# Quyans/SG-NeRF

Measured on AMD Instinct MI355X. Metric: rays/sec + ms/frame, 800×800×64 samples, ScanNet scene, 1/2/4/8 GPU, higher is better.
Workload: dtype f32 (3xf16 split MFMA, fp32 accumulate); 1 GPU; synth-room 800x800 rays x SR=64 samples, D=400, K=8, P=26, 1200000 neural points (BASELINE config 2, 1 frame per rank per step); rays_per_frame=640000, SR=64, K=8, D=400, points=1200000, parallelism=frame-sharded x1, outputs=rgb, ray mask, background transmission, coarse_point_opacity [R, SR]

## Files before the change

sg-nerf_amd/csrc/mlp_x3.hip:

```cpp
#include <cstdio>
#include <cstdlib>
#include <algorithm>
#include <cmath>
#include <utility>
#include <vector>

#include "agg_device.h"
#include "x3_split.h"

namespace sgn {
namespace {
namespace x3 {

constexpr int NW16 = 8, TPB16 = NW16 * 64;
constexpr int PAIR = 2048;
constexpr int SLOT_PAIRS = 32;
constexpr int SLOT = SLOT_PAIRS * PAIR;
constexpr int NSLOT = 2;
constexpr int PD = 2;
constexpr size_t PROJ_BYTES_PER_POINT = HID * 4;
struct XL {
    int ks, tp, np, kc;
    uint32_t off;
};
__host__ __device__ constexpr int nch(XL l) { return (l.ks + l.kc - 1) / l.kc; }
__host__ __device__ constexpr int nk(XL l, int c) { return l.ks - c * l.kc < l.kc ? l.ks - c * l.kc : l.kc; }

template <class Net>
struct Sched {
    static constexpr int layer_chunks(int l) { return Net::L[l].np * nch(Net::L[l]); }
    static constexpr int base(int l) { return l == 0 ? 0 : base(l - 1) + layer_chunks(l - 1); }
    static constexpr int total() { return base(Net::NL); }
    static constexpr int idx(int l, int p, int c) { return base(l) + p * nch(Net::L[l]) + c; }
    static constexpr int cl(int n, int l = 0) { return (l + 1 >= Net::NL || n < base(l + 1)) ? l : cl(n, l + 1); }
    static constexpr int cp(int n) { return (n - base(cl(n))) / nch(Net::L[cl(n)]); }
    static constexpr int cc(int n) { return (n - base(cl(n))) % nch(Net::L[cl(n)]); }
    static constexpr uint32_t off(int n) {
        return Net::L[cl(n)].off +
               (uint32_t)((cp(n) * Net::L[cl(n)].ks + cc(n) * Net::L[cl(n)].kc) * Net::L[cl(n)].tp) * PAIR;
    }
    static constexpr int pairs(int n) { return nk(Net::L[cl(n)], cc(n)) * Net::L[cl(n)].tp; }
};
struct X3B {
    h8 hi, lo;
};

__device__ __forceinline__ X3B split8(const float (&v)[8]) {
    const X3Pair p = split8_unit(v);
    return X3B{p.hi, p.lo};
}

__device__ __forceinline__ float lrelu_x3(float a) {
    float r = 0.01f * a;
    asm("v_max_f32 %0, %1, %0" : "+v"(r) : "v"(a));
    return r;
}
__device__ __forceinline__ X3B lrelu_split8(const float (&a)[8], float inv) {
    float v[8];
#pragma unroll
    for (int j = 0; j < 8; ++j) v[j] = lrelu_x3(a[j] * inv);
    return split8(v);
}

__device__ __forceinline__ void lds_dma_1k(const WBlob &wb, char *dst, int w, int lane, uint32_t soff) {
    asm volatile("" : "+s"(soff));
    __builtin_amdgcn_raw_ptr_buffer_load_lds(wb.rsrc, (__attribute__((address_space(3))) void *)(dst + w * 1024), 16,
                                             lane * 16 + w * 1024, soff, 0, 0);
}

template <class Net, int N, int NWv = NW16>
__device__ __forceinline__ void dma_chunk(const WBlob &wb, char *dst, int w, int lane, int) {
    using S = Sched<Net>;
    constexpr int nf = 2 * S::pairs(N);
    static_for<(nf + NWv - 1) / NWv>([&](auto jj) {
        constexpr int J = decltype(jj)::value;
        const int i = w + NWv * J;
        if (NWv * (J + 1) <= nf || i < nf)
            lds_dma_1k(wb, dst + NWv * J * 1024, w, lane, S::off(N) + (uint32_t)(NWv * J * 1024));
    });
}

template <class Net, int N, int J, int NWv = NW16>
__device__ __forceinline__ void dma_piece(const WBlob &wb, char *dst, int w, int lane, int) {
    using S = Sched<Net>;
    constexpr int nf = 2 * S::pairs(N);
    constexpr int PW = (nf + NWv - 1) / NWv;
    const int i = w * PW + J;
    if (nf % NWv == 0 || i < nf) {
        uint32_t soff = S::off(N) + (uint32_t)((J & ~3) * 1024);
        asm volatile("" : "+s"(soff));
        __builtin_amdgcn_raw_ptr_buffer_load_lds(wb.rsrc,
                                                 (__attribute__((address_space(3))) void *)(dst + (w * PW + (J & ~3)) * 1024),
                                                 16, lane * 16 + w * PW * 1024, soff, (J & 3) * 1024, 0);
    }
}
template <class Net, int N, int NWv = NW16>
constexpr int dma_pieces() { return (2 * Sched<Net>::pairs(N) + NWv - 1) / NWv; }

__device__ __forceinline__ int cur_slot(int s) { return s; }
__device__ __forceinline__ int dma_slot(int s) { return s ^ 1; }
__device__ __forceinline__ void chunk_exit(int &s, int) { s ^= 1; }

template <class Net, int N, int NWv = NW16, int VM = 0>
__device__ __forceinline__ void chunk_enter(const WBlob &, char *, int, int, int, int) {
    static_assert(VM >= 0 && VM < 64, "vmcnt range");
    if constexpr (VM == 0)
        asm volatile("s_waitcnt vmcnt(0)" ::: "memory");
    else
        __builtin_amdgcn_s_waitcnt((VM & 15) | (7 << 4) | (15 << 8) | ((VM >> 4) << 14));
    asm volatile("s_waitcnt lgkmcnt(0)" ::: "memory");
    __builtin_amdgcn_s_barrier();
}

struct NoHook {
    template <class C>
    __device__ void operator()(C) const {}
};
struct VmZero {
    static constexpr int vm(int) { return 0; }
};


template <int F>
__device__ __forceinline__ void sincos_f(float x, float &s, float &c) {
    sincos_acc(x * (float)(1 << F), s, c);
}
constexpr uint32_t OFF16_BASE = 0;
constexpr uint32_t OFF16_W0B = OFF16_BASE;
constexpr uint32_t OFF16_W1 = OFF16_W0B + 32 * PAIR;
constexpr uint32_t OFF16_W2 = OFF16_W1 + 128 * PAIR;
constexpr uint32_t OFF16_W3 = OFF16_W2 + 144 * PAIR;
constexpr uint32_t OFF16_W0A = OFF16_W3 + 128 * PAIR;
constexpr uint32_t OFF16_WB = OFF16_W0A + 112 * PAIR;
constexpr uint32_t OFF16_C0 = OFF16_WB + 176 * PAIR;
constexpr uint32_t OFF16_C1 = OFF16_C0 + 72 * PAIR;
constexpr uint32_t OFF16_C2 = OFF16_C1 + 32 * PAIR;
constexpr uint32_t OFF16_F32 = OFF16_C2 + 32 * PAIR;
constexpr int Y_B0 = 0, Y_B1 = 256, Y_B2 = 512, Y_B3 = 768, Y_WA = 1024, Y_BB = 1280, Y_BA = 1536, Y_INV = 1537;
constexpr int Y_CB0 = Y_INV + 8 + 3, Y_CB1 = Y_CB0 + 128, Y_CB2 = Y_CB1 + 128, Y_CW3 = Y_CB2 + 128, Y_CB3 = Y_CW3 + 384;
constexpr int N_Y32 = Y_CB3 + 4;
constexpr size_t BLOB_BYTES_ALL = OFF16_F32 + (size_t)N_Y32 * 4;
__host__ __device__ constexpr size_t blob_bytes_sg(int) { return BLOB_BYTES_ALL; }
static_assert(N_Y32 % 4 == 0, "fp32 section in 16-B units");

constexpr int NWR = 4;
constexpr int NSLR = NSLOT;
static_assert(NWR == 4, "row workgroup: 4 waves");
template <int SP_>
struct NetR16T {
    static constexpr int NW = NWR, SP = SP_;
    static constexpr int KC = SP_ / 16;
    static constexpr int NL = 4;
    static constexpr XL L[NL] = {{2, 16, 1, KC, OFF16_W0B}, {8, 16, 1, KC, OFF16_W1}, {9, 16, 1, KC, OFF16_W2},
                                 {8, 8, 2, 2 * KC, OFF16_W3}};
};
template <int KB, int SP_>
struct NetR16SGT {
    static constexpr int NW = NWR, SP = SP_;
    static constexpr int KC = SP_ / 16;
    static constexpr int NL = 5;
    static constexpr XL L[NL] = {{2, 16, 1, KC, OFF16_W0B}, {8, 16, 1, KC, OFF16_W1}, {KB, 16, 1, KC, OFF16_WB},
                                 {9, 16, 1, KC, OFF16_W2}, {8, 8, 2, 2 * KC, OFF16_W3}};
};
struct NetProj16 {
    static constexpr int NW = NW16, SP = SLOT_PAIRS;
    static constexpr int NL = 1;
    static constexpr XL L[NL] = {{7, 16, 1, 2, OFF16_W0A}};
};
constexpr int NWC = 8, SPC = NWC == 4 ? 16 : 32, KCC = SPC / 8;
static_assert(NWC == 4 || NWC == 8, "colour workgroup: 4 or 8 waves");
struct NetColor16 {
    static constexpr int NW = NWC, SP = SPC;
    static constexpr int NL = 3;
    static constexpr XL L[NL] = {{9, 8, 1, KCC, OFF16_C0}, {4, 8, 1, KCC, OFF16_C1}, {4, 8, 1, KCC, OFF16_C2}};
};
static_assert(Sched<NetR16T<16>>::total() == 27 && Sched<NetR16T<32>>::total() == 14 &&
                  Sched<NetR16T<32>>::pairs(9) == 16, "16x16 row stream");
static_assert(NWC == 4 ? Sched<NetColor16>::total() == 9 && Sched<NetColor16>::pairs(4) == 8
                       : Sched<NetColor16>::total() == 5 && Sched<NetColor16>::pairs(2) == 8, "16x16 colour stream");

__device__ __forceinline__ f32x4 mfma16(h8 a, h8 b, f32x4 c) {
    return __builtin_amdgcn_mfma_f32_16x16x32_f16(a, b, c, 0, 0, 0);
}

template <int NS>
struct X3S {
    X3B b[NS];
};

template <class Net, int L, bool TRANS = false, class Vm = VmZero, int P = 0, int AOFF = 0, bool PIPE = false,
          int NS, int NA, class SlotT, class InFn, class PostFn = NoHook, class EndFn = NoHook, class MidFn = NoHook>
__device__ __forceinline__ void run_layer_ns(const WBlob &wb, char *lds, SlotT &slot, int w, int lane, int lz,
                                             f32x4 (&acc)[NS][NA], InFn &&in, PostFn &&post = PostFn{},
                                             EndFn &&end = EndFn{}, MidFn &&mid = MidFn{}) {
    constexpr XL ly = Net::L[L];
    constexpr int TP = ly.tp;
    static_assert((TP == 16 || TP == 8) && P < ly.np, "passes of 16 or 8 output tiles");
    static_assert(AOFF + TP <= NA, "accumulator view");
    X3S<NS> Bn;
    if constexpr (PIPE) Bn = in(std::integral_constant<int, 0>{});
    static_for<nch(ly)>([&](auto cc) {
        constexpr int C = decltype(cc)::value;
        constexpr int N = Sched<Net>::idx(L, P, C), NN = (N + 1) % Sched<Net>::total();
        constexpr int NWv = Net::NW, SLOTv = Net::SP * PAIR;
        static_assert(nk(ly, C) * TP <= Net::SP, "chunk larger than a ring slot");
        chunk_enter<Net, N, NWv, Vm::vm(C)>(wb, lds, slot, w, lane, lz);
        post(cc);
        const char *sl = lds + cur_slot(slot) * SLOTv;
        char *dnext = lds + dma_slot(slot) * SLOTv;
        constexpr int NF = nk(ly, C) * TP;
        constexpr int PW = dma_pieces<Net, NN, NWv>();
        auto frag = [&](int f, int part) { return *(const h8 *)(sl + (2 * f + part) * 1024 + lane * 16); };
        h8 fh[PD], fl[PD];
#pragma unroll
        for (int f = 0; f < PD; ++f) {
            fh[f] = frag(f, 0);
            fl[f] = frag(f, 1);
        }
        __builtin_amdgcn_sched_group_barrier(0x100, 2 * PD, 0);
        static_for<nk(ly, C)>([&](auto kk) {
            constexpr int KK = decltype(kk)::value;
            constexpr int KS = C * ly.kc + KK;
            if constexpr (NS > 1 && KK > 0 && !PIPE) __builtin_amdgcn_sched_barrier(0);
            X3S<NS> B;
            if constexpr (PIPE) B = Bn;
            else B = in(std::integral_constant<int, KS>{});
            static_for<TP>([&](auto tt) {
                constexpr int t = decltype(tt)::value, F = KK * TP + t;
                const h8 Ah = fh[F % PD], Al = fl[F % PD];
                if constexpr (F + PD < NF) {
                    fh[F % PD] = frag(F + PD, 0);
                    fl[F % PD] = frag(F + PD, 1);
                }
#pragma unroll
                for (int s = 0; s < NS; ++s) {
                    f32x4 &c = acc[s][AOFF + t];
                    if constexpr (TRANS) {
                        c = mfma16(B.b[s].hi, Al, c);
                        c = mfma16(B.b[s].lo, Ah, c);
                        c = mfma16(B.b[s].hi, Ah, c);
                    } else {
                        c = mfma16(Al, B.b[s].hi, c);
                        c = mfma16(Ah, B.b[s].lo, c);
                        c = mfma16(Ah, B.b[s].hi, c);
                    }
                }
                constexpr int NSP = NF / 2 > 0 ? NF / 2 : 1;
                if constexpr (F < NSP) {
                    static_for<(F + 1) * PW / NSP - F * PW / NSP>([&](auto jj) {
                        dma_piece<Net, NN, F * PW / NSP + decltype(jj)::value, NWv>(wb, dnext, w, lane, lz);
                    });
                }
                mid(std::integral_constant<int, (C * ly.kc + KK) * TP + t>{});
                if constexpr (PIPE && t == TP / 2 - 1 && KS + 1 < ly.ks)
                    Bn = in(std::integral_constant<int, (KS + 1 < ly.ks ? KS + 1 : KS)>{});
                if constexpr (NS == 1) {
                    __builtin_amdgcn_sched_group_barrier(0x008, 1, 0);
                    __builtin_amdgcn_sched_group_barrier(0x100, 1, 0);
                    __builtin_amdgcn_sched_group_barrier(0x008, 1, 0);
                    __builtin_amdgcn_sched_group_barrier(0x100, 1, 0);
                    __builtin_amdgcn_sched_group_barrier(0x008, 1, 0);
                } else {
                    __builtin_amdgcn_sched_group_barrier(0x008, 3 * NS / 2, 0);
                    __builtin_amdgcn_sched_group_barrier(0x100, 1, 0);
                    __builtin_amdgcn_sched_group_barrier(0x008, 3 * NS - 3 * NS / 2, 0);
                    __builtin_amdgcn_sched_group_barrier(0x100, 1, 0);
                }
            });
        });
        __builtin_amdgcn_sched_barrier(0);
        end(cc);
        chunk_exit(slot, lane);
        __builtin_amdgcn_sched_barrier(0);
    });
}

template <class Net, int L, bool TRANS = false, class Vm = VmZero, int P = 0, class SlotT, class InFn,
          class PostFn = NoHook, class EndFn = NoHook, class MidFn = NoHook>
__device__ __forceinline__ void run_layer16(const WBlob &wb, char *lds, SlotT &slot, int w, int lane, int lz,
                                            f32x4 (&acc)[Net::L[L].tp], InFn &&in, PostFn &&post = PostFn{},
                                            EndFn &&end = EndFn{}, MidFn &&mid = MidFn{}) {
    constexpr int TP = Net::L[L].tp;
    run_layer_ns<Net, L, TRANS, Vm, P, 0>(wb, lds, slot, w, lane, lz, reinterpret_cast<f32x4(&)[1][TP]>(acc),
                                          [&](auto k) { return X3S<1>{{in(k)}}; }, post, end, mid);
}

template <bool ADD>
__device__ __forceinline__ void chain_out16(const f32x4 (&acc)[16], const f32x4 (&add)[16], float inv, X3B (&out)[8]) {
#pragma unroll
    for (int s = 0; s < 8; ++s) {
        float v[8];
#pragma unroll
        for (int j = 0; j < 8; ++j) {
            const float a = acc[2 * s + (j >> 2)][j & 3];
            const float y = ADD ? (a + add[2 * s + (j >> 2)][j & 3]) * inv : a * inv;
            v[j] = fmaxf(y, 0.01f * y);
        }
        out[s] = split8(v);
    }
}

struct Proj16Args {
    const float *emb;
    int64_t n;
    const void *blob;
    float *proj;
    const float *xyz, *color, *dir, *conf;
    float *rec;
    const int32_t *idx;
    const int64_t *n_dev;
};
constexpr int REC16_FLOATS = 16;
constexpr int Y_LDS_OFF = NSLOT * SLOT;
constexpr int PROJ16_LDS = Y_LDS_OFF + N_Y32 * 4;

__global__ __launch_bounds__(TPB16, 1) void k_point_proj16(Proj16Args a) {
    __shared__ __attribute__((aligned(16))) char lds[PROJ16_LDS];
    const int lane = threadIdx.x & 63, g = lane >> 4;
    const int w = __builtin_amdgcn_readfirstlane(threadIdx.x >> 6);
    const WBlob wb = make_blob(a.blob, BLOB_BYTES_ALL);
    {
        const float *src = (const float *)((const char *)a.blob + OFF16_F32);
        float *dst = (float *)(lds + Y_LDS_OFF);
        for (int i = threadIdx.x; i < N_Y32; i += TPB16) dst[i] = src[i];
    }
    __syncthreads();
    int slot = 0;
    dma_chunk<NetProj16, 0, NW16>(wb, lds, w, lane, 0);
    const int64_t n = a.idx ? min(*a.n_dev, a.n) : a.n;
    const int64_t ntile = (n + 16 * NW16 - 1) / (16 * NW16);
    for (int64_t tile = blockIdx.x; tile < ntile; tile += gridDim.x) {
        int lz = 0;
        asm volatile("" : "+s"(lz));
        const float *Yl = (const float *)(lds + lz + Y_LDS_OFF);
        const int64_t j = tile * (16 * NW16) + w * 16 + (lane & 15);
        const bool ok = j < n;
        const int64_t p = a.idx ? (ok ? (int64_t)a.idx[j] : 0) : j;
        float f8[8];
        {
            const f32x4 *e4 = (const f32x4 *)(a.emb + (ok ? p : 0) * 32 + 8 * g);
            const f32x4 u0 = e4[0], u1 = e4[1];
            f8[0] = u0[0]; f8[1] = u0[1]; f8[2] = u0[2]; f8[3] = u0[3];
            f8[4] = u1[0]; f8[5] = u1[1]; f8[6] = u1[2]; f8[7] = u1[3];
        }
        f32x4 acc[16];
#pragma unroll
        for (int t = 0; t < 16; ++t) acc[t] = *(const f32x4 *)(Yl + Y_B0 + 16 * t + 4 * g);
        auto in = [&](auto k) {
            constexpr int S = decltype(k)::value;
            float v[8];
            if constexpr (S == 0) {
#pragma unroll
                for (int j = 0; j < 8; ++j) v[j] = f8[j];
            } else {
                static_for<4>([&](auto jp) {
                    constexpr int q = 8 * (S - 1) + 2 * decltype(jp)::value, dl = q / 6, f = (q % 6) / 2;
                    float sv, cv;
                    sincos_f<f>(f8[dl], sv, cv);
                    v[2 * decltype(jp)::value] = sv;
                    v[2 * decltype(jp)::value + 1] = cv;
                });
            }
            return split8(v);
        };
        f32x4 q{};
        {
            const float *src = g == 0 ? a.xyz : g == 1 ? a.color : a.dir;
            const int64_t pc = ok ? p : 0;
            if (g < 3) q = f32x4{src[pc * 3], src[pc * 3 + 1], src[pc * 3 + 2], g == 0 ? a.conf[pc] : 0.f};
        }
        run_layer16<NetProj16, 0>(wb, lds + lz, slot, w, lane, lz, acc, in);
        if (ok) {
            float *dst = a.proj + p * HID + 4 * g;
#pragma unroll
            for (int t = 0; t < 16; ++t) *(f32x4 *)(dst + 16 * t) = acc[t];
            *(f32x4 *)(a.rec + p * REC16_FLOATS + 4 * g) = q;
        }
    }
    asm volatile("s_waitcnt vmcnt(0)" ::: "memory");
}

constexpr int WG16_SAMPLES = NWR * 2;
constexpr int TPBR = NWR * 64;
__host__ __device__ constexpr int yr_off(int sp) { return NSLR * sp * PAIR; }
__host__ __device__ constexpr int yt16_off(int sp) { return yr_off(sp) + N_Y32 * 4; }
__host__ __device__ constexpr int rows16_lds(int sp) { return yt16_off(sp) + 2 * 16 * 20 * 4; }
static_assert(2 * rows16_lds(16) <= 163840, "LDS budget (16x16 rows)");

template <bool PERS>
struct Rec16 {
    float p[3], col[3], dir[3], cf, l[3], v[3];
    float pp[PERS ? 3 : 1], pl[PERS ? 3 : 1];
};
constexpr int REC16_LOADS = 9;
template <bool PERS>
__device__ __forceinline__ Rec16<PERS> load_rec16(const AggArgs &a, const RowIdx &ix) {
    Rec16<PERS> r;
    const bool v = ix.sval;
    const int pid = ix.pid, s = ix.s, ray = ix.ray;
    const bool m = v && pid >= 0;
    const float *dummy = (const float *)a.blob;
    const f32x4 *rp = (const f32x4 *)(m ? a.rec + (int64_t)pid * REC16_FLOATS : dummy);
    const float *lp = v ? a.samp_locw + (int64_t)s * 3 : dummy;
    const float *vp = v ? a.raydir + (int64_t)ray * 3 : dummy;
    const f32x4 q0 = rp[0], q1 = rp[1], q2 = rp[2];
    float l3[3], v3[3];
#pragma unroll
    for (int c = 0; c < 3; ++c) {
        l3[c] = lp[c];
// ... 204 lines not shown
    else if constexpr (C == 7) return r.hi * 16.f;
    else return r.hi * (r.shi * (float)(1 << (2 * (C - 5))));
}
template <int S>
__device__ __forceinline__ X3B pe_dists16_k(const PeRow &r) {
    float x[4], u[8];
    static_for<4>([&](auto cc) { x[decltype(cc)::value] = pe_arg16<4 * S + decltype(cc)::value>(r); });
    const float m = fmaxf(fmaxf(__builtin_fabsf(x[0]), __builtin_fabsf(x[1])), fmaxf(__builtin_fabsf(x[2]), __builtin_fabsf(x[3])));
    if (__builtin_expect(__ballot(!(m < 1048576.f)) != 0, 0)) {
#pragma unroll
        for (int q = 0; q < 4; ++q) sincosf(x[q], &u[2 * q], &u[2 * q + 1]);
    } else {
#pragma unroll
        for (int q = 0; q < 4; ++q) sincos_acc_fast(x[q], u[2 * q], u[2 * q + 1]);
    }
    return split8(u);
}

struct Epi16 {
    float wsa[4], wsb[4];
    float ap[4];
    float fsv[4];
    float *fs_dst;
    bool fs_have;
    float inv3;
};

struct Tiles {
    int first, end, step;
};
__device__ __forceinline__ Tiles grid_tiles(int ntiles) { return Tiles{(int)blockIdx.x, ntiles, (int)gridDim.x}; }

template <int KB, bool PERS, bool SAVE = false, int NS = 1, int SP = 16>
__global__ __launch_bounds__(TPBR, NS == 1 ? 8 / NWR : 1) void k_rows16(AggArgs a) {
    using Net = std::conditional_t<(KB > 0), NetR16SGT<KB, SP>, NetR16T<SP>>;
    constexpr int YR_OFF = yr_off(SP), YT16_OFF = yt16_off(SP), ROWS16_LDS = rows16_lds(SP);
    constexpr int LB = 2, L2 = KB ? 3 : 2, L3 = KB ? 4 : 3;
    constexpr int NBP = KB > 8 ? KB - 8 : 0;
    constexpr int WGS = WG16_SAMPLES * NS;
    __shared__ __attribute__((aligned(16))) char lds[ROWS16_LDS];
    const int lane = threadIdx.x & 63;
    const int g = lane >> 4, r = lane & 15, kk = lane & 7, sc = r >> 3;
    const int w = __builtin_amdgcn_readfirstlane(threadIdx.x >> 6);
    const int nslots = a.slot_n[0];
    const Cam cam = load_cam(a.campos, a.rot);
    const WBlob wb = make_blob(a.blob, BLOB_BYTES_ALL);
    const float *proj = (const float *)a.proj;
    {
        const float *src = (const float *)((const char *)a.blob + OFF16_F32);
        float *dst = (float *)(lds + YR_OFF);
        for (int i = threadIdx.x; i < N_Y32; i += TPBR) dst[i] = src[i];
        {
            float *yt = (float *)(lds + YT16_OFF);
            for (int i = threadIdx.x; i < 512; i += TPBR) {
                const int which = i >> 8, u = i & 255, t = u >> 4, rr = u & 15;
                yt[which * 320 + rr * 20 + t] = src[(which ? Y_WA : Y_B3) + 16 * t + rr];
            }
        }
    }
    __syncthreads();
    int slot = 0;
    dma_chunk<Net, 0, NWR>(wb, lds, w, lane, 0);
    const Tiles xt = grid_tiles((nslots + WGS - 1) / WGS);
    RowIdx nx[NS];
    Rec16<PERS> rnext[NS];
#pragma unroll
    for (int q = 0; q < NS; ++q) {
        nx[q] = row_index16(a, xt.first * WGS + w * 2 * NS + 2 * q + sc, nslots, kk);
        rnext[q] = load_rec16<PERS>(a, nx[q]);
    }
    auto load_p = [&](int pid, f32x4 (&dst)[16]) {
        const float *src = proj + (int64_t)(pid < 0 ? 0 : pid) * HID + 4 * g;
#pragma unroll
        for (int t = 0; t < 16; ++t) dst[t] = *(const f32x4 *)(src + 16 * t);
    };
    f32x4 accA[NS][16], accB[NS][16];
#pragma unroll
    for (int q = 0; q < NS; ++q) load_p(nx[q].pid, pick<(KB > 0)>(accB[q], accA[q]));

    auto epi_begin = [&](Epi16 &e, const char *ldsi, float wgt, int nA, int nB, int2 ce, bool ok) {
        const float inv3 = ((const float *)(ldsi + YR_OFF))[Y_INV + 3];
#pragma unroll
        for (int i = 0; i < 4; ++i) {
            const float wi = __builtin_bit_cast(float, __builtin_amdgcn_ds_bpermute((4 * g + i) * 4, __builtin_bit_cast(int, wgt)));
            const bool inA = 4 * (g & 1) + i < nA;
            const float ws = wi;
            e.wsa[i] = inA ? ws : 0.f;
            e.wsb[i] = inA ? 0.f : ws;
            e.ap[i] = 0.f;
        }
        e.fs_have = ((g & 1) ? nB > 0 : nA > 0) && ok;
        e.inv3 = inv3;
        e.fs_dst = (float *)a.fs + (int64_t)((uint32_t)((g & 1) ? ce.y : ce.x) & 0x0FFFFFFFu) * HID + r;
    };
    auto epi_step = [&](Epi16 &e, const char *ldsi, const f32x4 (&ac)[16], auto tc) {
        constexpr int T = decltype(tc)::value;
        const float wau = ((const float *)(ldsi + YT16_OFF))[320 + r * 20 + T];
        float fa = 0.f, fb = 0.f;
#pragma unroll
        for (int i = 0; i < 4; ++i) {
            const float hv = lrelu_x3(__builtin_fmaf(ac[T][i], e.inv3, ((const float *)(ldsi + YT16_OFF))[r * 20 + T]));
            e.ap[i] = __builtin_fmaf(wau, hv, e.ap[i]);
            fa = __builtin_fmaf(e.wsa[i], hv, fa);
            fb = __builtin_fmaf(e.wsb[i], hv, fb);
        }
        permlane16_swap(fa, fb);
        e.fsv[T & 3] = fa + fb;
        if constexpr ((T & 3) == 3) {
            if (e.fs_have) {
#pragma unroll
                for (int u = 0; u < 4; ++u) e.fs_dst[16 * (T - 3 + u)] = e.fsv[u];
            }
        }
    };
    auto epi_end = [&](Epi16 &e, const char *ldsi, int nA, int nB, int s_ix) {
        const float ba = ((const float *)(ldsi + YR_OFF))[Y_BA];
        float xr[4];
#pragma unroll
        for (int i = 0; i < 4; ++i) {
            float x = dpp_sum8(e.ap[i]);
            x += __builtin_bit_cast(float, __builtin_amdgcn_mov_dpp(__builtin_bit_cast(int, x), 0x128, 0xF, 0xF, true));
            xr[i] = x;
        }
        const int q4 = r & 3;
        const float spm = softplus((q4 == 0 ? xr[0] : q4 == 1 ? xr[1] : q4 == 2 ? xr[2] : xr[3]) + ba - 1.f);
        const int spi = __builtin_bit_cast(int, spm);
        const float sp4[4] = {__builtin_bit_cast(float, __builtin_amdgcn_mov_dpp(spi, 0x00, 0xF, 0xF, true)),
                              __builtin_bit_cast(float, __builtin_amdgcn_mov_dpp(spi, 0x55, 0xF, 0xF, true)),
                              __builtin_bit_cast(float, __builtin_amdgcn_mov_dpp(spi, 0xAA, 0xF, 0xF, true)),
                              __builtin_bit_cast(float, __builtin_amdgcn_mov_dpp(spi, 0xFF, 0xF, 0xF, true))};
        float asa = 0.f, asb = 0.f;
#pragma unroll
        for (int i = 0; i < 4; ++i) {
            asa = __builtin_fmaf(e.wsa[i], sp4[i], asa);
            asb = __builtin_fmaf(e.wsb[i], sp4[i], asb);
        }
        permlane16_swap(asa, asb);
        const float as = asa + asb;
        const int s_of = __builtin_amdgcn_ds_bpermute((8 * (g >> 1) + ((g & 1) ? (nA > 4 ? nA : 4) : 0)) * 4, s_ix);
        if (r == 0 && ((g & 1) ? nB > 0 : nA > 0)) a.feat[(int64_t)s_of * 4 + 0] = as;
    };

    for (int tile = xt.first; tile < xt.end; tile += xt.step) {
        const int base = tile * WGS;
        int lz = 0;
        asm volatile("" : "+s"(lz));
        char *ldsi = lds + lz;
        const float *Yl = (const float *)(ldsi + YR_OFF);
        RowIdx ix[NS];
        Row16 rw[NS];
        int nslot[NS], nA[NS], nB[NS];
        uint64_t mrowA[NS], mrowB[NS];
        int64_t vrow[NS];
        X3B ext[NS];
        const int hsh = 8 * (g >> 1);
#pragma unroll
        for (int q = 0; q < NS; ++q) {
            const int hslot = base + w * 2 * NS + 2 * q + sc;
            nslot[q] = tile + xt.step < xt.end ? hslot + xt.step * WGS : nslots;
            ix[q] = nx[q];
            const bool m = ix[q].pid >= 0;
            const Rec16<PERS> rc = rnext[q];
            mrowA[q] = __ballot(ix[q].sval && ix[q].a);
            mrowB[q] = __ballot(ix[q].sval && !ix[q].a);
            const int nA0 = __popc((uint32_t)mrowA[q] & 0xFFu), nA1 = __popc(((uint32_t)mrowA[q] >> 8) & 0xFFu);
            const bool waveB = (mrowB[q] & 0xFFFFull) != 0;
            rw[q] = row_math16<PERS>(cam, rc, m, ix[q].a, sc ? nA1 : nA0, waveB);
            nA[q] = __popcll((mrowA[q] >> hsh) & 0xFFull);
            nB[q] = __popcll((mrowB[q] >> hsh) & 0xFFull);
            vrow[q] = -1;
            if (SAVE && ix[q].sval && m) {
                const int e = a.rows[(int64_t)hslot * 8 + kk];
                vrow[q] = a.row_off ? (int64_t)a.row_off[e >> 3] + (e & 7) : pidx_of(a, e);
            }
            if ((a.blend || a.wnorm) && ix[q].sval) {
                const int64_t v = pidx_of(a, a.rows[(int64_t)hslot * 8 + kk]);
                if (a.blend && g == 0) a.blend[v] = rw[q].wgt;
                if (a.wnorm && g == 1) a.wnorm[v] = rw[q].wn;
            }
            {
                const bool e = g == 0 && m;
                float u[8];
                u[0] = e ? rc.col[0] : 0.f; u[1] = e ? rc.col[1] : 0.f; u[2] = e ? rc.col[2] : 0.f;
                u[3] = e ? __fsub_rn(rc.dir[0], rc.v[0]) : 0.f;
                u[4] = e ? __fsub_rn(rc.dir[1], rc.v[1]) : 0.f;
                u[5] = e ? __fsub_rn(rc.dir[2], rc.v[2]) : 0.f;
                u[6] = e ? __fadd_rn(__fadd_rn(__fmul_rn(rc.dir[0], rc.v[0]), __fmul_rn(rc.dir[1], rc.v[1])),
                                     __fmul_rn(rc.dir[2], rc.v[2])) : 0.f;
                u[7] = 0.f;
                ext[q] = split8(u);
            }
        }
        auto chain_k = [&](int q, const f32x4 (&ac)[16], float inv, auto kc, float *zsave = nullptr) {
            constexpr int S = decltype(kc)::value;
            float v[8];
#pragma unroll
            for (int j = 0; j < 8; ++j) v[j] = ac[2 * S + (j >> 2)][j & 3];
            if constexpr (SAVE) {
                if (zsave && vrow[q] >= 0) {
                    float *zr = zsave + vrow[q] * HID + 4 * g;
                    *(f32x4 *)(zr + 32 * S) = f32x4{v[0] * inv, v[1] * inv, v[2] * inv, v[3] * inv};
                    *(f32x4 *)(zr + 32 * S + 16) = f32x4{v[4] * inv, v[5] * inv, v[6] * inv, v[7] * inv};
                }
            }
            return lrelu_split8(v, inv);
        };
        auto bias_init = [&](f32x4 (&ac)[16], int yb) {
#pragma unroll
            for (int t = 0; t < 16; ++t) ac[t] = *(const f32x4 *)(Yl + yb + 16 * t + 4 * g);
        };
        {
            PeRow pr[NS];
#pragma unroll
            for (int q = 0; q < NS; ++q) {
                pr[q] = pe_row16(rw[q].d, g);
                if constexpr (KB > 0) {
#pragma unroll
                    for (int t = 0; t < 16; ++t) accA[q][t] = accB[q][t];
                }
            }
            run_layer_ns<Net, 0, false, std::conditional_t<SAVE, VmZero, VmL0<NS>>, 0, 0, !SAVE>(
                wb, ldsi, slot, w, lane, lz, accA, [&](auto k) {
                    X3S<NS> o;
#pragma unroll
                    for (int q = 0; q < NS; ++q) o.b[q] = pe_dists16_k<decltype(k)::value>(pr[q]);
                    return o;
                }, NoHook{});
        }
        const float inv0 = Yl[Y_INV + 0], inv1 = Yl[Y_INV + 1], inv2 = Yl[Y_INV + 2], inv7 = Yl[Y_INV + 7];
#pragma unroll
        for (int q = 0; q < NS; ++q) bias_init(accB[q], Y_B1);
        int v_next[NS];
        run_layer_ns<Net, 1, false, VmZero, 0, 0, !SAVE>(wb, ldsi, slot, w, lane, lz, accB, [&](auto k) {
            X3S<NS> o;
#pragma unroll
            for (int q = 0; q < NS; ++q) o.b[q] = chain_k(q, accA[q], inv0, k, a.z1);
            return o;
        }, [&](auto c) {
            if constexpr (decltype(c)::value == 0) {
#pragma unroll
                for (int q = 0; q < NS; ++q) v_next[q] = nslot[q] < nslots ? a.rows[(int64_t)nslot[q] * 8 + kk] : -1;
            }
        });
        if constexpr (KB > 0) {
            X3B bpv[NS][NBP > 0 ? NBP : 1];
            if constexpr (NBP > 0) {
#pragma unroll
                for (int q = 0; q < NS; ++q) {
                    const float *src = a.bpnet32 + (int64_t)(ix[q].pid >= 0 ? ix[q].pid : 0) * (NBP * 32) + 8 * g;
#pragma unroll
                    for (int j = 0; j < NBP; ++j) {
                        const f32x4 u0 = *(const f32x4 *)(src + 32 * j), u1 = *(const f32x4 *)(src + 32 * j + 4);
                        const float v[8] = {u0[0], u0[1], u0[2], u0[3], u1[0], u1[1], u1[2], u1[3]};
                        bpv[q][j] = split8(v);
                    }
                }
            }
#pragma unroll
            for (int q = 0; q < NS; ++q) bias_init(accA[q], Y_BB);
            run_layer_ns<Net, LB>(wb, ldsi, slot, w, lane, lz, accA, [&](auto k) {
                constexpr int K = decltype(k)::value;
                X3S<NS> o;
#pragma unroll
                for (int q = 0; q < NS; ++q) {
                    if constexpr (K < 8) o.b[q] = chain_k(q, accB[q], inv1, k, a.z2);
                    else o.b[q] = bpv[q][K - 8];
                }
                return o;
            }, NoHook{});
        }
        auto &in2 = pick<(KB > 0)>(accA, accB);
        auto &acc2 = pick<(KB > 0)>(accB, accA);
        const float inv_in2 = KB > 0 ? inv7 : inv1;
#pragma unroll
        for (int q = 0; q < NS; ++q) bias_init(acc2[q], Y_B2);
        run_layer_ns<Net, L2, false, VmZero, 0, 0, !SAVE>(wb, ldsi, slot, w, lane, lz, acc2, [&](auto k) {
            constexpr int K = decltype(k)::value;
            X3S<NS> o;
#pragma unroll
            for (int q = 0; q < NS; ++q) {
                if constexpr (K < 8) o.b[q] = chain_k(q, in2[q], inv_in2, k, KB > 0 ? a.zb : a.z2);
                else o.b[q] = ext[q];
            }
            return o;
        }, [&](auto c) {
            constexpr int C = decltype(c)::value;
            if constexpr (C == 0) {
#pragma unroll
                for (int q = 0; q < NS; ++q) {
                    nx[q].sval = v_next[q] >= 0;
                    nx[q].s = nx[q].sval ? v_next[q] >> 3 : 0;
                    nx[q].a = (v_next[q] & 7) == kk;
                    nx[q].pid = nx[q].sval ? a.pidx[pidx_of(a, v_next[q])] : -1;
                    nx[q].ray = nx[q].sval ? a.samp_ray[nx[q].s] : 0;
                }
            }
        });
        auto &acc = in2;
#pragma unroll
        for (int q = 0; q < NS; ++q)
#pragma unroll
            for (int t = 0; t < 16; ++t) acc[q][t] = f32x4{};
        int2 ce[NS];
        int eslot[NS];
#pragma unroll
        for (int q = 0; q < NS; ++q) {
            ce[q] = make_int2(0, 0);
            eslot[q] = base + w * 2 * NS + 2 * q + (g >> 1);
        }
        auto first_chunk_loads = [&](auto c) {
            if constexpr (decltype(c)::value == 0) {
#pragma unroll
                for (int q = 0; q < NS; ++q) {
                    rnext[q] = load_rec16<PERS>(a, nx[q]);
                    ce[q] = *(const int2 *)(a.slots + (eslot[q] < nslots ? eslot[q] : 0));
                }
            }
        };
        Epi16 e[NS];
        {
            X3B in3[NS][8];
            run_layer_ns<Net, L3, true, std::conditional_t<SAVE, VmZero, VmL3P0<NS>>, 0, 0, !SAVE>(
                wb, ldsi, slot, w, lane, lz, acc, [&](auto k) {
                    constexpr int K = decltype(k)::value;
                    X3S<NS> o;
#pragma unroll
                    for (int q = 0; q < NS; ++q) {
                        in3[q][K] = chain_k(q, acc2[q], inv2, k, a.z3);
                        o.b[q] = in3[q][K];
                    }
                    return o;
                }, NoHook{}, first_chunk_loads);
#pragma unroll
            for (int q = 0; q < NS; ++q) epi_begin(e[q], ldsi, rw[q].wgt, nA[q], nB[q], ce[q], eslot[q] < nslots);
            run_layer_ns<Net, L3, true, VmZero, 1, 8>(wb, ldsi, slot, w, lane, lz, acc, [&](auto k) {
                X3S<NS> o;
#pragma unroll
                for (int q = 0; q < NS; ++q) o.b[q] = in3[q][decltype(k)::value];
                return o;
            }, NoHook{}, NoHook{}, [&](auto f) {
                constexpr int F = decltype(f)::value;
                if constexpr ((F & 7) == 7) {
#pragma unroll
                    for (int q = 0; q < NS; ++q) epi_step(e[q], ldsi, acc[q], std::integral_constant<int, F / 8>{});
                }
            });
        }
#pragma unroll
        for (int q = 0; q < NS; ++q) {
            asm volatile("" : "+v"(nx[q].s), "+v"(nx[q].pid), "+v"(nx[q].ray));
#pragma unroll
            for (int c = 0; c < 3; ++c) {
                asm volatile("" : "+v"(rnext[q].p[c]), "+v"(rnext[q].col[c]), "+v"(rnext[q].dir[c]), "+v"(rnext[q].l[c]),
                             "+v"(rnext[q].v[c]));
                if constexpr (PERS) asm volatile("" : "+v"(rnext[q].pp[c]), "+v"(rnext[q].pl[c]));
            }
            asm volatile("" : "+v"(rnext[q].cf));
        }
        {
            constexpr int NE = 8, PPE = 16 / NE;
            static_for<NE>([&](auto tc) {
                constexpr int J = decltype(tc)::value;
#pragma unroll
                for (int q = 0; q < NS; ++q) {
                    const float *psrc = proj + (int64_t)(nx[q].pid < 0 ? 0 : nx[q].pid) * HID + 4 * g;
#pragma unroll
                    for (int u = 0; u < PPE; ++u) acc2[q][PPE * J + u] = *(const f32x4 *)(psrc + 16 * (PPE * J + u));
                    epi_step(e[q], ldsi, acc[q], std::integral_constant<int, (16 - NE) + J>{});
                }
            });
#pragma unroll
            for (int q = 0; q < NS; ++q) epi_end(e[q], ldsi, nA[q], nB[q], ix[q].s);
        }
    }
    asm volatile("s_waitcnt vmcnt(0)" ::: "memory");
}

int perm16(int p) { return 16 * ((p & 7) >> 2) + 4 * (p >> 3) + (p & 3); }
int col_chain16(int ks, int p) { return 32 * ks + perm16(p); }
int col_l2_16(int ks, int p) { return ks < 8 ? col_chain16(ks, p) : (p < 7 ? 256 + p : -1); }
int col_l0b16(int s, int p) {
    const int g = p >> 3, c = 4 * s + ((p & 7) >> 1);
    int comp, f;
    if (c < 5) {
        comp = g;
        f = c;
    } else {
        comp = 4 + (g & 1);
        f = c == 5 ? (g >= 2) : c == 6 ? 2 + (g >= 2) : 4;
        if (c == 7 && g >= 2) return -1;
    }
    return 224 + 2 * (5 * comp + f) + (p & 1);
}
int col_proj16(int s, int p) { return s == 0 ? p : 32 + 48 * (p >> 3) + 8 * (s - 1) + (p & 7); }
int col_bp16(int ks, int p) { return ks < 8 ? col_chain16(ks, p) : 256 + 32 * (ks - 8) + p; }
int col_c016(int ks, int p) {
    if (ks < 8) return 32 * ks + p;
    const int g = p >> 3, f = (p & 7) >> 1;
    return g < 3 ? 256 + ((p & 1) ? 12 : 0) + 4 * g + f : -1;
}

template <typename ColFn>
void pack_pairs16(_Float16 *dst, const float *W, int n_out, int n_in, int KS, int shift, ColFn col, int NT = 16,
                  int NP = 1) {
    const float sc = ldexpf(1.f, shift);
    const int TPP = NT / NP;
    for (int t = 0; t < NT; ++t)
        for (int ks = 0; ks < KS; ++ks) {
            const size_t f = ((size_t)(t / TPP) * KS + ks) * TPP + t % TPP;
            for (int lane = 0; lane < 64; ++lane)
                for (int e = 0; e < 8; ++e) {
                    const int row = 16 * t + (lane & 15);
                    const int c = col(ks, 8 * (lane >> 4) + e);
                    const float v = (row < n_out && c >= 0 && c < n_in) ? W[(size_t)row * n_in + c] * sc : 0.f;
                    const _Float16 hi = (_Float16)v;
                    const _Float16 lo = (_Float16)(v - (float)hi);
                    dst[((2 * f) * 64 + lane) * 8 + e] = hi;
                    dst[((2 * f + 1) * 64 + lane) * 8 + e] = lo;
                }
        }
}

enum Y32Kind { YK_ZERO = 0, YK_W = 1, YK_B = 2, YK_BS = 3, YK_INV = 4, YK_ONE = 5, YK_WINV = 6, YK_BS_OR_B = 7 };
template <class Pairs, class F32>
void layout_blob16(int ksb, int bpnet_dim, Pairs &&pairs, F32 &&f32) {
    pairs(OFF16_W0B, 0, 256, 284, 2, col_l0b16, 16, 1);
    pairs(OFF16_W1, 1, 256, 256, 8, col_chain16, 16, 1);
    pairs(OFF16_W2, 2, 256, 263, 9, col_l2_16, 16, 1);
    pairs(OFF16_W3, 3, 256, 256, 8, col_chain16, 16, 2);
    pairs(OFF16_W0A, 0, 256, 284, 7, col_proj16, 16, 1);
    for (int u = 0; u < HID; ++u) {
        f32(Y_B0 + u, YK_BS, 0, u);
        f32(Y_B1 + u, YK_BS, 1, u);
        f32(Y_B2 + u, YK_BS, 2, u);
        f32(Y_B3 + u, YK_B, 3, u);
        f32(Y_WA + u, YK_W, 4, u);
    }
    f32(Y_BA, YK_B, 4, 0);
    const int li[7] = {0, 1, 2, 3, 5, 6, 7};
    for (int i = 0; i < 7; ++i) f32(Y_INV + i, YK_INV, li[i], 0);
    f32(Y_INV + 7, ksb > 0 ? YK_INV : YK_ONE, 9, 0);
    if (ksb > 0) {
        pairs(OFF16_WB, 9, 256, 256 + bpnet_dim, 8 + bpnet_dim / 32, col_bp16, 16, 1);
        for (int u = 0; u < HID; ++u) f32(Y_BB + u, YK_BS, 9, u);
    }
    pairs(OFF16_C0, 5, 128, 280, 9, col_c016, 8, 1);
    pairs(OFF16_C1, 6, 128, 128, 4, col_chain16, 8, 1);
    pairs(OFF16_C2, 7, 128, 128, 4, col_chain16, 8, 1);
    for (int u = 0; u < 128; ++u) {
        f32(Y_CB0 + u, YK_BS, 5, u);
        f32(Y_CB1 + u, YK_BS, 6, u);
        f32(Y_CB2 + u, YK_BS, 7, u);
        for (int c = 0; c < 3; ++c) f32(Y_CW3 + 128 * c + u, YK_W, 8, c * 128 + u);
    }
    for (int c = 0; c < 3; ++c) f32(Y_CB3 + c, YK_B, 8, c);
}

void pack_blob16(int ksb, int bpnet_dim, const float *const *w, const float *const *b, const int *s, int sb,
                 uint8_t *blob) {
    auto shift = [&](int L) { return L == 9 ? sb : s[L]; };
    float *Y = (float *)(blob + OFF16_F32);
    layout_blob16(ksb, bpnet_dim,
                  [&](uint32_t off, int L, int n_out, int n_in, int KS, auto col, int NT, int NP) {
                      pack_pairs16((_Float16 *)(blob + off), w[L], n_out, n_in, KS, shift(L), col, NT, NP);
                  },
                  [&](int yi, int kind, int L, int e) {
                      float v = 0.f;
                      switch (kind) {
                          case YK_W: v = w[L][e]; break;
                          case YK_B: v = b[L][e]; break;
                          case YK_BS: v = b[L][e] * ldexpf(1.f, shift(L)); break;
                          case YK_INV: v = ldexpf(1.f, -shift(L)); break;
                          case YK_ONE: v = 1.f; break;
                          case YK_WINV: v = w[L][e] * ldexpf(1.f, -shift(3)); break;
                          default: break;
                      }
                      Y[yi] = v;
                  });
}

void index_blob16(int ksb, int bpnet_dim, int32_t *i16, size_t n16, int32_t *i32, size_t n32) {
    for (size_t i = 0; i < n16; ++i) i16[i] = -1;
    for (size_t i = 0; i < n32; ++i) i32[i] = 0;
    layout_blob16(ksb, bpnet_dim,
                  [&](uint32_t off, int L, int n_out, int n_in, int KS, auto col, int NT, int NP) {
                      const int TPP = NT / NP;
                      int32_t *dst = i16 + off / 2;
                      for (int t = 0; t < NT; ++t)
                          for (int ks = 0; ks < KS; ++ks) {
                              const size_t f = ((size_t)(t / TPP) * KS + ks) * TPP + t % TPP;
                              for (int lane = 0; lane < 64; ++lane)
                                  for (int e = 0; e < 8; ++e) {
                                      const int row = 16 * t + (lane & 15);
                                      const int c = col(ks, 8 * (lane >> 4) + e);
                                      const bool ok = row < n_out && c >= 0 && c < n_in;
                                      const int32_t code = ok ? (L << 20) | (row * n_in + c) : -1;
                                      dst[((2 * f) * 64 + lane) * 8 + e] = code;
                                      dst[((2 * f + 1) * 64 + lane) * 8 + e] = ok ? code | (1 << 30) : -1;
                                  }
                          }
                  },
                  [&](int yi, int kind, int L, int e) { i32[yi] = (kind << 26) | (L << 20) | e; });
}
struct ColorArgs {
    const int32_t *counters, *work, *samp_ray;
    const float *raydir;
    const void *blob;
    const float *fs;
    float *feat;
    int32_t *range_flag;
    int32_t item0, n_items;
};
constexpr int YC_OFF = NSLOT * SPC * PAIR, TPBC = NWC * 64;
constexpr int COL16_LDS = YC_OFF + N_Y32 * 4;
static_assert(COL16_LDS * (8 / NWC) <= 163840, "LDS budget (colour, 8 / NWC workgroups per CU)");

__global__ __launch_bounds__(TPBC, 8 / NWC) void k_color16(ColorArgs a) {
    __shared__ __attribute__((aligned(16))) char lds[COL16_LDS];
    const int lane = threadIdx.x & 63;
    const int g = lane >> 4, r = lane & 15;
    const int w = __builtin_amdgcn_readfirstlane(threadIdx.x >> 6);
    const int nwork = a.counters[1];
    const int end = min(nwork, a.item0 + a.n_items);
    const WBlob wb = make_blob(a.blob, BLOB_BYTES_ALL);
    {
        const float *src = (const float *)((const char *)a.blob + OFF16_F32);
        float *dst = (float *)(lds + YC_OFF);
        for (int i = threadIdx.x; i < N_Y32; i += TPBC) dst[i] = src[i];
    }
    __syncthreads();
    int slot = 0;
    dma_chunk<NetColor16, 0, NWC>(wb, lds, w, lane, 0);
    f32x4 fr[16];
    float vd[3];
    int sn = 0, rn = 0;
    auto load_q = [&](auto qc, int item) {
        constexpr int Q = decltype(qc)::value;
        const bool ok = item < end;
        const f32x4 *row = (const f32x4 *)(a.fs + (int64_t)(ok ? item - a.item0 : 0) * HID + 8 * g) + 16 * Q;
        f32x4 t0, t1, t2, t3;
        asm volatile("global_load_dwordx4 %0, %1, off" : "=v"(t0) : "v"(row));
        asm volatile("global_load_dwordx4 %0, %1, off offset:16" : "=v"(t1) : "v"(row));
        asm volatile("global_load_dwordx4 %0, %1, off offset:128" : "=v"(t2) : "v"(row));
        asm volatile("global_load_dwordx4 %0, %1, off offset:144" : "=v"(t3) : "v"(row));
        fr[4 * Q] = t0;
        fr[4 * Q + 1] = t1;
        fr[4 * Q + 2] = t2;
        fr[4 * Q + 3] = t3;
    };
    auto load_sid = [&](int item) { sn = item < end ? a.work[item] : 0; };
    auto load_ray = [&]() { rn = a.samp_ray[sn]; };
    auto load_dir = [&]() {
#pragma unroll
        for (int c = 0; c < 3; ++c) vd[c] = a.raydir[(int64_t)rn * 3 + c];
    };
    {
        const int item = a.item0 + blockIdx.x * (16 * NWC) + w * 16 + r;
        load_sid(item);
        load_q(std::integral_constant<int, 0>{}, item);
        load_q(std::integral_constant<int, 1>{}, item);
        load_q(std::integral_constant<int, 2>{}, item);
        asm volatile("s_waitcnt vmcnt(0)" ::: "memory");
    }
    load_ray();
    for (int base = a.item0 + blockIdx.x * (16 * NWC); base < end; base += gridDim.x * (16 * NWC)) {
        int lz = 0;
        asm volatile("" : "+s"(lz));
        char *ldsi = lds + lz;
        const float *Yl = (const float *)(ldsi + YC_OFF);
        const int item = base + w * 16 + r;
        const bool sval = item < end;
        const int s = sn;
        auto bias = [&](f32x4 (&ac)[8], int yb) {
#pragma unroll
            for (int t = 0; t < 8; ++t) ac[t] = *(const f32x4 *)(Yl + yb + 16 * t + 4 * g);
        };
        auto chain = [&](const f32x4 (&ac)[8], float inv, auto kc) {
            constexpr int S = decltype(kc)::value;
            float v[8];
#pragma unroll
            for (int j = 0; j < 8; ++j) v[j] = ac[2 * S + (j >> 2)][j & 3];
            return lrelu_split8(v, inv);
        };
        f32x4 c0[8], c1[8];
        bias(c0, Y_CB0);
        run_layer16<NetColor16, 0>(wb, ldsi, slot, w, lane, lz, c0, [&](auto k) {
            constexpr int K = decltype(k)::value;
            float v[8];
            if constexpr (K < 8) {
                f32x4 u0 = fr[2 * K], u1 = fr[2 * K + 1];
                asm volatile("" : "+v"(u0), "+v"(u1));
                v[0] = u0[0]; v[1] = u0[1]; v[2] = u0[2]; v[3] = u0[3];
                v[4] = u1[0]; v[5] = u1[1]; v[6] = u1[2]; v[7] = u1[3];
            } else {
                const float x = g == 0 ? vd[0] : g == 1 ? vd[1] : vd[2];
                float y[4];
#pragma unroll
                for (int f = 0; f < 4; ++f) y[f] = x * (float)(1 << f);
                const float m = fmaxf(fmaxf(__builtin_fabsf(y[0]), __builtin_fabsf(y[1])),
                                      fmaxf(__builtin_fabsf(y[2]), __builtin_fabsf(y[3])));
                if (__builtin_expect(__ballot(!(m < 1048576.f)) != 0, 0)) {
#pragma unroll
                    for (int f = 0; f < 4; ++f) sincosf(y[f], &v[2 * f], &v[2 * f + 1]);
                } else {
#pragma unroll
                    for (int f = 0; f < 4; ++f) sincos_acc_fast(y[f], v[2 * f], v[2 * f + 1]);
                }
            }
            return split8(v);
        }, [&](auto c) {
            constexpr int C = decltype(c)::value;
            if constexpr (C == 0) {
                load_q(std::integral_constant<int, 3>{}, item);
                load_dir();
            }
            if constexpr (C == 1) load_q(std::integral_constant<int, 0>{}, item + gridDim.x * (16 * NWC));
        });
        bias(c1, Y_CB1);
        const float inv4 = Yl[Y_INV + 4], inv5 = Yl[Y_INV + 5], inv6 = Yl[Y_INV + 6];
        run_layer16<NetColor16, 1>(wb, ldsi, slot, w, lane, lz, c1, [&](auto k) { return chain(c0, inv4, k); },
                                   [&](auto c) {
                                       if constexpr (decltype(c)::value == 0) {
                                           load_q(std::integral_constant<int, 1>{}, item + gridDim.x * (16 * NWC));
                                           load_sid(item + gridDim.x * (16 * NWC));
                                       }
                                   });
        bias(c0, Y_CB2);
        run_layer16<NetColor16, 2>(wb, ldsi, slot, w, lane, lz, c0, [&](auto k) { return chain(c1, inv5, k); },
                                   [&](auto c) {
                                       if constexpr (decltype(c)::value == 0) {
                                           load_q(std::integral_constant<int, 2>{}, item + gridDim.x * (16 * NWC));
                                           load_ray();
                                       }
                                   });
        float o[3] = {0.f, 0.f, 0.f};
#pragma unroll
        for (int t = 0; t < 8; ++t) {
            f32x4 wc[3];
#pragma unroll
            for (int c = 0; c < 3; ++c) wc[c] = *(const f32x4 *)(Yl + Y_CW3 + 128 * c + 16 * t + 4 * g);
#pragma unroll
            for (int i = 0; i < 4; ++i) {
                const float y = c0[t][i] * inv6;
                const float hv = lrelu_x3(y);
#pragma unroll
                for (int c = 0; c < 3; ++c) o[c] = __builtin_fmaf(wc[c][i], hv, o[c]);
            }
        }
        bool fin = true;
#pragma unroll
        for (int c = 0; c < 3; ++c) {
            float x = o[c] + __shfl_xor(o[c], 16);
            x += __shfl_xor(x, 32);
// ... 248 lines not shown
```

Before: 27.49 million rays/s.

## Pack block-3 extra-input K-step as single-fragment MFMA with hi/lo spread across lanes

The ninth K-step of layer 2 (the 7 extra inputs: colour, direction terms) previously used the 3xf16 split with hi and lo weight fragments, needing three MFMAs and two fragment loads. This change re-lays out the weights and activations across the K dimension, placing hi and lo products in different lane groups. That lets the chunk run as a single MFMA per tile with one weight fragment, which halves that chunk's DMA and LDS traffic. Packing, indexing and scheduling are extended to handle the 'single' chunk, and compile-time asserts check that the offsets still line up.

```diff
diff --git a/sg-nerf_amd/csrc/mlp_x3.hip b/sg-nerf_amd/csrc/mlp_x3.hip
--- a/sg-nerf_amd/csrc/mlp_x3.hip
+++ b/sg-nerf_amd/csrc/mlp_x3.hip
@@ -22,6 +22,7 @@
 struct XL {
     int ks, tp, np, kc;
     uint32_t off;
+    int one = 0;
 };
 __host__ __device__ constexpr int nch(XL l) { return (l.ks + l.kc - 1) / l.kc; }
 __host__ __device__ constexpr int nk(XL l, int c) { return l.ks - c * l.kc < l.kc ? l.ks - c * l.kc : l.kc; }
@@ -40,6 +41,12 @@
                (uint32_t)((cp(n) * Net::L[cl(n)].ks + cc(n) * Net::L[cl(n)].kc) * Net::L[cl(n)].tp) * PAIR;
     }
     static constexpr int pairs(int n) { return nk(Net::L[cl(n)], cc(n)) * Net::L[cl(n)].tp; }
+    static constexpr bool single(int n) { return Net::L[cl(n)].one && cc(n) == nch(Net::L[cl(n)]) - 1; }
+    static constexpr int frags(int n) { return single(n) ? pairs(n) : 2 * pairs(n); }
+    static constexpr bool single_ok(int l = 0) {
+        return l >= Net::NL || ((!Net::L[l].one || (Net::L[l].np == 1 && (Net::L[l].ks - 1) % Net::L[l].kc == 0)) &&
+                                single_ok(l + 1));
+    }
 };
 struct X3B {
     h8 hi, lo;
@@ -71,7 +78,7 @@
 template <class Net, int N, int NWv = NW16>
 __device__ __forceinline__ void dma_chunk(const WBlob &wb, char *dst, int w, int lane, int) {
     using S = Sched<Net>;
-    constexpr int nf = 2 * S::pairs(N);
+    constexpr int nf = S::frags(N);
     static_for<(nf + NWv - 1) / NWv>([&](auto jj) {
         constexpr int J = decltype(jj)::value;
         const int i = w + NWv * J;
@@ -83,7 +90,7 @@
 template <class Net, int N, int J, int NWv = NW16>
 __device__ __forceinline__ void dma_piece(const WBlob &wb, char *dst, int w, int lane, int) {
     using S = Sched<Net>;
-    constexpr int nf = 2 * S::pairs(N);
+    constexpr int nf = S::frags(N);
     constexpr int PW = (nf + NWv - 1) / NWv;
     const int i = w * PW + J;
     if (nf % NWv == 0 || i < nf) {
@@ -95,7 +102,7 @@
     }
 }
 template <class Net, int N, int NWv = NW16>
-constexpr int dma_pieces() { return (2 * Sched<Net>::pairs(N) + NWv - 1) / NWv; }
+constexpr int dma_pieces() { return (Sched<Net>::frags(N) + NWv - 1) / NWv; }
 
 __device__ __forceinline__ int cur_slot(int s) { return s; }
 __device__ __forceinline__ int dma_slot(int s) { return s ^ 1; }
@@ -129,7 +136,8 @@
 constexpr uint32_t OFF16_W0B = OFF16_BASE;
 constexpr uint32_t OFF16_W1 = OFF16_W0B + 32 * PAIR;
 constexpr uint32_t OFF16_W2 = OFF16_W1 + 128 * PAIR;
-constexpr uint32_t OFF16_W3 = OFF16_W2 + 144 * PAIR;
+constexpr uint32_t OFF16_W2X = OFF16_W2 + 128 * PAIR;
+constexpr uint32_t OFF16_W3 = OFF16_W2X + 16 * (PAIR / 2);
 constexpr uint32_t OFF16_W0A = OFF16_W3 + 128 * PAIR;
 constexpr uint32_t OFF16_WB = OFF16_W0A + 112 * PAIR;
 constexpr uint32_t OFF16_C0 = OFF16_WB + 176 * PAIR;
@@ -151,7 +159,7 @@
     static constexpr int NW = NWR, SP = SP_;
     static constexpr int KC = SP_ / 16;
     static constexpr int NL = 4;
-    static constexpr XL L[NL] = {{2, 16, 1, KC, OFF16_W0B}, {8, 16, 1, KC, OFF16_W1}, {9, 16, 1, KC, OFF16_W2},
+    static constexpr XL L[NL] = {{2, 16, 1, KC, OFF16_W0B}, {8, 16, 1, KC, OFF16_W1}, {9, 16, 1, KC, OFF16_W2, 1},
                                  {8, 8, 2, 2 * KC, OFF16_W3}};
 };
 template <int KB, int SP_>
@@ -160,7 +168,7 @@
     static constexpr int KC = SP_ / 16;
     static constexpr int NL = 5;
     static constexpr XL L[NL] = {{2, 16, 1, KC, OFF16_W0B}, {8, 16, 1, KC, OFF16_W1}, {KB, 16, 1, KC, OFF16_WB},
-                                 {9, 16, 1, KC, OFF16_W2}, {8, 8, 2, 2 * KC, OFF16_W3}};
+                                 {9, 16, 1, KC, OFF16_W2, 1}, {8, 8, 2, 2 * KC, OFF16_W3}};
 };
 struct NetProj16 {
     static constexpr int NW = NW16, SP = SLOT_PAIRS;
@@ -176,6 +184,13 @@
 };
 static_assert(Sched<NetR16T<16>>::total() == 27 && Sched<NetR16T<32>>::total() == 14 &&
                   Sched<NetR16T<32>>::pairs(9) == 16, "16x16 row stream");
+static_assert(Sched<NetR16T<16>>::single(18) && Sched<NetR16T<16>>::frags(18) == 16 &&
+                  Sched<NetR16T<16>>::off(18) == OFF16_W2X && !Sched<NetR16T<16>>::single(17) &&
+                  Sched<NetR16T<16>>::off(19) == OFF16_W3 && Sched<NetR16T<32>>::single(9) &&
+                  Sched<NetR16T<32>>::off(9) == OFF16_W2X && Sched<NetR16T<16>>::single_ok() &&
+                  Sched<NetR16T<32>>::single_ok() && Sched<NetR16SGT<11, 16>>::single_ok() &&
+                  Sched<NetR16SGT<8, 16>>::off(26) == OFF16_W2X && Sched<NetR16SGT<8, 16>>::single(26),
+              "block3.0's extras: the chunk of 16 single fragments after its 128 pairs");
 static_assert(NWC == 4 ? Sched<NetColor16>::total() == 9 && Sched<NetColor16>::pairs(4) == 8
                        : Sched<NetColor16>::total() == 5 && Sched<NetColor16>::pairs(2) == 8, "16x16 colour stream");
 
@@ -203,21 +218,25 @@
         constexpr int C = decltype(cc)::value;
         constexpr int N = Sched<Net>::idx(L, P, C), NN = (N + 1) % Sched<Net>::total();
         constexpr int NWv = Net::NW, SLOTv = Net::SP * PAIR;
+        constexpr bool ONE = Sched<Net>::single(N);
         static_assert(nk(ly, C) * TP <= Net::SP, "chunk larger than a ring slot");
+        static_assert(!(ONE && TRANS), "single fragments are A operands");
         chunk_enter<Net, N, NWv, Vm::vm(C)>(wb, lds, slot, w, lane, lz);
         post(cc);
         const char *sl = lds + cur_slot(slot) * SLOTv;
         char *dnext = lds + dma_slot(slot) * SLOTv;
         constexpr int NF = nk(ly, C) * TP;
         constexpr int PW = dma_pieces<Net, NN, NWv>();
-        auto frag = [&](int f, int part) { return *(const h8 *)(sl + (2 * f + part) * 1024 + lane * 16); };
+        auto frag = [&](int f, int part) {
+            return *(const h8 *)(sl + (ONE ? f : 2 * f + part) * 1024 + lane * 16);
+        };
         h8 fh[PD], fl[PD];
 #pragma unroll
         for (int f = 0; f < PD; ++f) {
             fh[f] = frag(f, 0);
-            fl[f] = frag(f, 1);
-        }
-        __builtin_amdgcn_sched_group_barrier(0x100, 2 * PD, 0);
+            if constexpr (!ONE) fl[f] = frag(f, 1);
+        }
+        __builtin_amdgcn_sched_group_barrier(0x100, (ONE ? 1 : 2) * PD, 0);
         static_for<nk(ly, C)>([&](auto kk) {
             constexpr int KK = decltype(kk)::value;
             constexpr int KS = C * ly.kc + KK;
@@ -227,15 +246,17 @@
             else B = in(std::integral_constant<int, KS>{});
             static_for<TP>([&](auto tt) {
                 constexpr int t = decltype(tt)::value, F = KK * TP + t;
-                const h8 Ah = fh[F % PD], Al = fl[F % PD];
+                const h8 Ah = fh[F % PD], Al = ONE ? Ah : fl[F % PD];
                 if constexpr (F + PD < NF) {
                     fh[F % PD] = frag(F + PD, 0);
-                    fl[F % PD] = frag(F + PD, 1);
+                    if constexpr (!ONE) fl[F % PD] = frag(F + PD, 1);
                 }
 #pragma unroll
                 for (int s = 0; s < NS; ++s) {
                     f32x4 &c = acc[s][AOFF + t];
-                    if constexpr (TRANS) {
+                    if constexpr (ONE) {
+                        c = mfma16(Ah, B.b[s].hi, c);
+                    } else if constexpr (TRANS) {
                         c = mfma16(B.b[s].hi, Al, c);
                         c = mfma16(B.b[s].lo, Ah, c);
                         c = mfma16(B.b[s].hi, Ah, c);
@@ -254,7 +275,10 @@
                 mid(std::integral_constant<int, (C * ly.kc + KK) * TP + t>{});
                 if constexpr (PIPE && t == TP / 2 - 1 && KS + 1 < ly.ks)
                     Bn = in(std::integral_constant<int, (KS + 1 < ly.ks ? KS + 1 : KS)>{});
-                if constexpr (NS == 1) {
+                if constexpr (ONE) {
+                    __builtin_amdgcn_sched_group_barrier(0x008, NS, 0);
+                    __builtin_amdgcn_sched_group_barrier(0x100, 1, 0);
+                } else if constexpr (NS == 1) {
                     __builtin_amdgcn_sched_group_barrier(0x008, 1, 0);
                     __builtin_amdgcn_sched_group_barrier(0x100, 1, 0);
                     __builtin_amdgcn_sched_group_barrier(0x008, 1, 0);
@@ -765,7 +789,7 @@
         int nslot[NS], nA[NS], nB[NS];
         uint64_t mrowA[NS], mrowB[NS];
         int64_t vrow[NS];
-        X3B ext[NS];
+        h8 ext[NS];
         const int hsh = 8 * (g >> 1);
 #pragma unroll
         for (int q = 0; q < NS; ++q) {
@@ -792,7 +816,7 @@
                 if (a.wnorm && g == 1) a.wnorm[v] = rw[q].wn;
             }
             {
-                const bool e = g == 0 && m;
+                const bool e = g != 3 && m;
                 float u[8];
                 u[0] = e ? rc.col[0] : 0.f; u[1] = e ? rc.col[1] : 0.f; u[2] = e ? rc.col[2] : 0.f;
                 u[3] = e ? __fsub_rn(rc.dir[0], rc.v[0]) : 0.f;
@@ -801,7 +825,8 @@
                 u[6] = e ? __fadd_rn(__fadd_rn(__fmul_rn(rc.dir[0], rc.v[0]), __fmul_rn(rc.dir[1], rc.v[1])),
                                      __fmul_rn(rc.dir[2], rc.v[2])) : 0.f;
                 u[7] = 0.f;
-                ext[q] = split8(u);
+                const X3B x = split8(u);
+                ext[q] = g == 1 ? x.lo : x.hi;
             }
         }
         auto chain_k = [&](int q, const f32x4 (&ac)[16], float inv, auto kc, float *zsave = nullptr) {
@@ -893,7 +918,7 @@
 #pragma unroll
             for (int q = 0; q < NS; ++q) {
                 if constexpr (K < 8) o.b[q] = chain_k(q, in2[q], inv_in2, k, KB > 0 ? a.zb : a.z2);
-                else o.b[q] = ext[q];
+                else o.b[q] = X3B{ext[q], ext[q]};
             }
             return o;
         }, [&](auto c) {
@@ -991,7 +1016,8 @@
 
 int perm16(int p) { return 16 * ((p & 7) >> 2) + 4 * (p >> 3) + (p & 3); }
 int col_chain16(int ks, int p) { return 32 * ks + perm16(p); }
-int col_l2_16(int ks, int p) { return ks < 8 ? col_chain16(ks, p) : (p < 7 ? 256 + p : -1); }
+constexpr int COL_LO = 1 << 30;
+int col_l2x16(int p) { return (p & 7) < 7 && p < 24 ? (256 + (p & 7)) | (p >= 16 ? COL_LO : 0) : -1; }
 int col_l0b16(int s, int p) {
     const int g = p >> 3, c = 4 * s + ((p & 7) >> 1);
     int comp, f;
@@ -1034,12 +1060,23 @@
         }
 }
 
+template <typename ColFn, typename Fn>
+void walk_singles16(int NT, ColFn col, Fn &&fn) {
+    for (int t = 0; t < NT; ++t)
+        for (int lane = 0; lane < 64; ++lane)
+            for (int e = 0; e < 8; ++e) {
+                const int c = col(8 * (lane >> 4) + e);
+                fn(((size_t)t * 64 + lane) * 8 + e, 16 * t + (lane & 15), c < 0 ? -1 : c & ~COL_LO, c >= 0 && (c & COL_LO));
+            }
+}
+
 enum Y32Kind { YK_ZERO = 0, YK_W = 1, YK_B = 2, YK_BS = 3, YK_INV = 4, YK_ONE = 5, YK_WINV = 6, YK_BS_OR_B = 7 };
-template <class Pairs, class F32>
-void layout_blob16(int ksb, int bpnet_dim, Pairs &&pairs, F32 &&f32) {
+template <class Pairs, class Singles, class F32>
+void layout_blob16(int ksb, int bpnet_dim, Pairs &&pairs, Singles &&singles, F32 &&f32) {
     pairs(OFF16_W0B, 0, 256, 284, 2, col_l0b16, 16, 1);
     pairs(OFF16_W1, 1, 256, 256, 8, col_chain16, 16, 1);
-    pairs(OFF16_W2, 2, 256, 263, 9, col_l2_16, 16, 1);
+    pairs(OFF16_W2, 2, 256, 263, 8, col_chain16, 16, 1);
+    singles(OFF16_W2X, 2, 256, 263, col_l2x16, 16);
     pairs(OFF16_W3, 3, 256, 256, 8, col_chain16, 16, 2);
     pairs(OFF16_W0A, 0, 256, 284, 7, col_proj16, 16, 1);
     for (int u = 0; u < HID; ++u) {
@@ -1076,6 +1113,15 @@
     layout_blob16(ksb, bpnet_dim,
                   [&](uint32_t off, int L, int n_out, int n_in, int KS, auto col, int NT, int NP) {
                       pack_pairs16((_Float16 *)(blob + off), w[L], n_out, n_in, KS, shift(L), col, NT, NP);
+                  },
+                  [&](uint32_t off, int L, int n_out, int n_in, auto col, int NT) {
+                      _Float16 *dst = (_Float16 *)(blob + off);
+                      const float sc = ldexpf(1.f, shift(L));
+                      walk_singles16(NT, col, [&](size_t i, int row, int c, bool lo) {
+                          const float v = (row < n_out && c >= 0 && c < n_in) ? w[L][(size_t)row * n_in + c] * sc : 0.f;
+                          const _Float16 hi = (_Float16)v;
+                          dst[i] = lo ? (_Float16)(v - (float)hi) : hi;
+                      });
                   },
                   [&](int yi, int kind, int L, int e) {
                       float v = 0.f;
@@ -1112,6 +1158,13 @@
                                       dst[((2 * f + 1) * 64 + lane) * 8 + e] = ok ? code | (1 << 30) : -1;
                                   }
                           }
+                  },
+                  [&](uint32_t off, int L, int n_out, int n_in, auto col, int NT) {
+                      int32_t *dst = i16 + off / 2;
+                      walk_singles16(NT, col, [&](size_t i, int row, int c, bool lo) {
+                          const bool ok = row < n_out && c >= 0 && c < n_in;
+                          dst[i] = ok ? ((L << 20) | (row * n_in + c)) | (lo ? 1 << 30 : 0) : -1;
+                      });
                   },
                   [&](int yi, int kind, int L, int e) { i32[yi] = (kind << 26) | (L << 20) | e; });
 }
```

After: 27.71 million rays/s, median of 3. No clear change (+0.8%).
